# apple/swift-homomorphic-encryption

Measured on NVIDIA H100. Metric: BFV ct*ct mults/sec at N=8192, 4 coefficient moduli, higher is better.
Workload: dtype u64

## Files before the change

### swift-homomorphic-encryption_b200/csrc/ntt_fast.cu

```cuda
#include <cuda.h>

#include <mutex>

#include <algorithm>
#include "kernels.cuh"
#include "ntt_fast.cuh"

namespace hecuda {
using namespace fast;

constexpr int kMaxRowList = 2 * (kMaxL + 1) * kMaxL;
struct RowList {
    int rows_per_poly;
    int count;
    unsigned short row[kMaxRowList];
    unsigned short slot[kMaxRowList];
    unsigned char flags[kMaxRowList];
    unsigned short src_row[kMaxRowList];
    long long src_poly_stride;
};

__device__ __forceinline__ u32 smem_u32(const void *p) { return (u32)__cvta_generic_to_shared(p); }
__device__ __forceinline__ void mbar_init(u64 *bar, int count) {
    asm volatile("mbarrier.init.shared::cta.b64 [%0], %1;" ::"r"(smem_u32(bar)), "r"(count) : "memory");
    asm volatile("fence.mbarrier_init.release.cluster;" ::: "memory");
}
__device__ __forceinline__ void mbar_arrive_expect_tx(u64 *bar, u32 bytes) {
    asm volatile("mbarrier.arrive.expect_tx.shared::cta.b64 _, [%0], %1;" ::"r"(smem_u32(bar)), "r"(bytes) : "memory");
}
__device__ __forceinline__ void mbar_wait(u64 *bar, u32 parity) {
    asm volatile(
        "{\n\t.reg .pred done;\n\t"
        "WAIT_%=:\n\t"
        "mbarrier.try_wait.parity.shared::cta.b64 done, [%0], %1;\n\t"
        "@!done bra WAIT_%=;\n\t}" ::"r"(smem_u32(bar)),
        "r"(parity)
        : "memory");
}
__device__ __forceinline__ void tma_load_1d(void *smem_dst, const void *gmem_src, u32 bytes, u64 *bar) {
    asm volatile("cp.async.bulk.shared::cluster.global.mbarrier::complete_tx::bytes [%0], [%1], %2, [%3];" ::"r"(smem_u32(smem_dst)),
                 "l"(gmem_src), "r"(bytes), "r"(smem_u32(bar))
                 : "memory");
}
__device__ __forceinline__ void tma_load_box(void *smem_dst, const CUtensorMap *map, int line, u64 *bar) {
    asm volatile("cp.async.bulk.tensor.2d.shared::cluster.global.tile.mbarrier::complete_tx::bytes [%0], [%1, {%2, %3}], [%4];" ::"r"(
                     smem_u32(smem_dst)),
                 "l"(map), "r"(0), "r"(line), "r"(smem_u32(bar))
                 : "memory");
}
__device__ __forceinline__ void tma_store_box(const CUtensorMap *map, int line, const void *smem_src) {
    asm volatile("cp.async.bulk.tensor.2d.global.shared::cta.tile.bulk_group [%0, {%1, %2}], [%3];" ::"l"(map), "r"(0), "r"(line),
                 "r"(smem_u32(smem_src))
                 : "memory");
}
__device__ __forceinline__ void tma_prefetch_box(const CUtensorMap *map, int line) {
    asm volatile("cp.async.bulk.prefetch.tensor.2d.L2.global.tile [%0, {%1, %2}];" ::"l"(map), "r"(0), "r"(line) : "memory");
}
__device__ __forceinline__ void tma_commit() { asm volatile("cp.async.bulk.commit_group;" ::: "memory"); }
template <int PENDING>
__device__ __forceinline__ void tma_store_wait_read() { asm volatile("cp.async.bulk.wait_group.read %0;" ::"n"(PENDING) : "memory"); }
__device__ __forceinline__ void tma_store_wait_all() { asm volatile("cp.async.bulk.wait_group 0;" ::: "memory"); }
__device__ __forceinline__ void fence_proxy_async_smem() { asm volatile("fence.proxy.async.shared::cta;" ::: "memory"); }

template <int LOGN, int CLS, int K>
__device__ __forceinline__ void fwd_row_pass(u64 (&x)[16], u64 *sm, int tau, const RowMod &m, bool reduce_in) {
    constexpr int P = plan_passes(LOGN), C = fwd_c(LOGN, K), LB = fwd_lb(LOGN, K);
    load_smem<LOGN, LB, C>(x, sm, tau);
    if (K == 0 && reduce_in) {
#pragma unroll
        for (int r = 0; r < 16; ++r) x[r] = barrett64(x[r], 0 - m.np, m.slot->mu1);
    }
    fwd_pass<LOGN, LB, C, CLS>(x, tau, m);
    if (K == P - 1) fwd_finish<CLS>(x, m);
    store_smem<LOGN, LB, C>(x, sm, tau);
}
template <int LOGN, int CLS>
__device__ __forceinline__ void fwd_row(u64 *sm, int tau, const RowMod &m, bool reduce_in) {
    constexpr int P = plan_passes(LOGN);
    u64 x[16];
    fwd_row_pass<LOGN, CLS, 0>(x, sm, tau, m, reduce_in);
    __syncthreads();
    fwd_row_pass<LOGN, CLS, 1>(x, sm, tau, m, false);
    __syncthreads();
    if (P == 4) {
        fwd_row_pass<LOGN, CLS, (P == 4 ? 2 : 1)>(x, sm, tau, m, false);
        __syncthreads();
    }
    fwd_row_pass<LOGN, CLS, P - 1>(x, sm, tau, m, false);
}

template <int LOGN, int CLS, int K>
__device__ __forceinline__ void inv_row_pass(u64 (&x)[16], u64 *sm, int tau, const RowMod &m) {
    constexpr int C = inv_c(LOGN, K), LB = inv_lb(LOGN, K);
    load_smem<LOGN, LB, C>(x, sm, tau);
    if (narrow_like(CLS) && K > 0 && inv_reduce_at(LOGN, K)) inv_reduce(x, m);
    inv_pass<LOGN, LB, C, CLS, inv_bound_in(LOGN, K)>(x, tau, m);
    if (K == plan_passes(LOGN) - 1 && m.partial) {
        if (CLS == kSmall) {
#pragma unroll
            for (int r = 0; r < 16; ++r) x[r] = csub32((u32)x[r], (u32)(0 - m.np));
        } else {
            reduce_small16(x, m);
        }
    }
    store_smem<LOGN, LB, C>(x, sm, tau);
}
template <int LOGN, int CLS>
__device__ __forceinline__ void inv_row(u64 *sm, int tau, const RowMod &m) {
    constexpr int P = plan_passes(LOGN);
    u64 x[16];
    inv_row_pass<LOGN, CLS, 0>(x, sm, tau, m);
    __syncthreads();
    inv_row_pass<LOGN, CLS, 1>(x, sm, tau, m);
    __syncthreads();
    if (P == 4) {
        inv_row_pass<LOGN, CLS, (P == 4 ? 2 : 1)>(x, sm, tau, m);
        __syncthreads();
    }
    inv_row_pass<LOGN, CLS, P - 1>(x, sm, tau, m);
}

template <int LOGN, unsigned CLASSES>
__device__ __forceinline__ void fwd_row_of(int cls, u64 *sm, int tau, const RowMod &m, bool reduce_in) {
    if (has_class(CLASSES, kNarrowH) && cls == kNarrowH) fwd_row<LOGN, kNarrowH>(sm, tau, m, reduce_in);
    else if (has_class(CLASSES, kNarrow) && narrow_like(cls)) fwd_row<LOGN, kNarrow>(sm, tau, m, reduce_in);
    else if (has_class(CLASSES, kSmall) && cls == kSmall) fwd_row<LOGN, kSmall>(sm, tau, m, reduce_in);
    else if (has_class(CLASSES, kMid) && cls == kMid) fwd_row<LOGN, kMid>(sm, tau, m, reduce_in);
    else if (has_class(CLASSES, kWide)) fwd_row<LOGN, kWide>(sm, tau, m, reduce_in);
}
template <int LOGN, unsigned CLASSES>
__device__ __forceinline__ void inv_row_of(int cls, u64 *sm, int tau, const RowMod &m) {
    if (has_class(CLASSES, kNarrowH) && cls == kNarrowH) inv_row<LOGN, kNarrowH>(sm, tau, m);
    else if (has_class(CLASSES, kNarrow) && narrow_like(cls)) inv_row<LOGN, kNarrow>(sm, tau, m);
    else if (has_class(CLASSES, kSmall) && cls == kSmall) inv_row<LOGN, kSmall>(sm, tau, m);
    else if (has_class(CLASSES, kMid) && cls == kMid) inv_row<LOGN, kMid>(sm, tau, m);
    else if (has_class(CLASSES, kWide)) inv_row<LOGN, kWide>(sm, tau, m);
}

HE_HD constexpr int ntt_row_buffers(int logn) { return logn == 13 ? 2 : 1; }

template <int LOGN>
constexpr size_t ntt_smem_bytes() {
    constexpr int B = ntt_row_buffers(LOGN);
    return sizeof(u64) * B * ((size_t)1 << LOGN) + sizeof(ulonglong2) * ((size_t)1 << (LOGN - 4)) + sizeof(u64) * (B + 1);
}

constexpr int ntt_min_ctas(int logn) { return logn == 13 ? 1 : 1024 / ((1 << logn) / 16); }

template <int LOGN, bool INVERSE, unsigned CLASSES>
__global__ void __launch_bounds__((1 << LOGN) / 16, ntt_min_ctas(LOGN))
    ntt_rows_kernel(const __grid_constant__ CUtensorMap map_in, const __grid_constant__ CUtensorMap map_out,
                    const ModSlot *__restrict__ slots, const __grid_constant__ RowList rl, const int polys,
                    const int scale_mode) {
    extern __shared__ __align__(1024) u64 smem[];
    constexpr int kLines = (1 << LOGN) / kLineWords;
    constexpr int kBoxes = kLines > kBoxLines ? kLines / kBoxLines : 1;
    constexpr int kLinesPerBox = kLines / kBoxes;
    constexpr u32 kRowBytes = (u32)sizeof(u64) << LOGN, kTwBytes = (u32)sizeof(ulonglong2) << (LOGN - 4);
    constexpr int B = ntt_row_buffers(LOGN), AHEAD = B > 1 ? 1 : 0;
    ulonglong2 *tw_cache = reinterpret_cast<ulonglong2 *>(smem + B * (1 << LOGN));
    u64 *bar_row = reinterpret_cast<u64 *>(tw_cache + (1 << (LOGN - 4)));
    u64 *bar_tw = bar_row + B;
    const int tau = threadIdx.x;
    const int tasks = polys * rl.count;
    auto in_line = [&](int t) {
        const int w = t / polys, p = t - w * polys;
        const int64_t word = INVERSE ? ((int64_t)p * rl.rows_per_poly + rl.row[w]) << LOGN
                                     : (int64_t)p * rl.src_poly_stride + ((int64_t)rl.src_row[w] << LOGN);
        return (int)(word >> 4);
    };
    auto load_row = [&](int t, int buf) {
        mbar_arrive_expect_tx(&bar_row[buf], kRowBytes);
        const int line = in_line(t);
        u64 *dst = smem + buf * (1 << LOGN);
#pragma unroll
        for (int b = 0; b < kBoxes; ++b) tma_load_box(dst + b * kLinesPerBox * kLineWords, &map_in, line + b * kLinesPerBox, &bar_row[buf]);
    };
    if (tau == 0) {
        if (smem_u32(smem) & 1023) __trap();
#pragma unroll
        for (int b = 0; b < B; ++b) mbar_init(&bar_row[b], 1);
        mbar_init(bar_tw, 1);
        if (AHEAD && (int)blockIdx.x < tasks) load_row(blockIdx.x, 0);
    }
    __syncthreads();
    u32 phase_row = 0, phase_tw = 0;
    int cached_slot = -1;
    int buf = 0;
    for (int task = blockIdx.x; task < tasks; task += gridDim.x) {
        const int which = task / polys;
        const int poly = task - which * polys;
        const int flags = rl.flags[which];
        const int slot = rl.slot[which];
        const ModSlot &S = slots[slot];
        u64 *sm = smem + buf * (1 << LOGN);
        const int64_t out_word = ((int64_t)poly * rl.rows_per_poly + rl.row[which]) << LOGN;
        const bool new_slot = slot != cached_slot;
        cached_slot = slot;
        if (tau == 0) {
            if (new_slot) {
                mbar_arrive_expect_tx(bar_tw, kTwBytes);
                tma_load_1d(tw_cache, INVERSE ? S.itw : S.tw, kTwBytes, bar_tw);
            }
            const int fill = task + AHEAD * gridDim.x;
            if (fill < tasks) {
                tma_store_wait_read<B - 1 - AHEAD>();
                load_row(fill, (buf + AHEAD) % B);
            }
            const int next = fill + gridDim.x;
            if (next < tasks) {
                const int line = in_line(next);
#pragma unroll
                for (int b = 0; b < kBoxes; ++b) tma_prefetch_box(&map_in, line + b * kLinesPerBox);
            }
        }
        const int cls = flags & 7;
        RowMod m;
        m.np = 0 - S.p;
        m.kp = (cls == kWide || cls == kSmall) ? 2 * S.p : 4 * S.p;
        m.tw = nullptr;
        m.tw_s = smem_u32(tw_cache);
        m.slot = &S;
        m.scale_mode = INVERSE ? scale_mode : -1;
        m.partial = INVERSE && (flags & 16) != 0;
        if (new_slot) {
            mbar_wait(bar_tw, phase_tw);
            phase_tw ^= 1;
        }
        mbar_wait(&bar_row[buf], (phase_row >> buf) & 1);
        phase_row ^= 1u << buf;
        if (INVERSE) inv_row_of<LOGN, CLASSES>(cls, sm, tau, m);
        else fwd_row_of<LOGN, CLASSES>(cls, sm, tau, m, (flags & 8) != 0);
        fence_proxy_async_smem();
        __syncthreads();
        if (tau == 0) {
            const int line = (int)(out_word >> 4);
#pragma unroll
            for (int b = 0; b < kBoxes; ++b) tma_store_box(&map_out, line + b * kLinesPerBox, sm + b * kLinesPerBox * kLineWords);
            tma_commit();
        }
        buf = buf + 1 == B ? 0 : buf + 1;
    }
    if (tau == 0) tma_store_wait_all();
}

__device__ __forceinline__ u32 cluster_ctarank() {
    u32 r;
    asm("mov.u32 %0, %%cluster_ctarank;" : "=r"(r));
    return r;
}
__device__ __forceinline__ int cluster_id_x() {
    u32 r;
    asm("mov.u32 %0, %%clusterid.x;" : "=r"(r));
    return (int)r;
}
__device__ __forceinline__ int cluster_count_x() {
    u32 r;
    asm("mov.u32 %0, %%nclusterid.x;" : "=r"(r));
    return (int)r;
}
__device__ __forceinline__ void cluster_arrive() { asm volatile("barrier.cluster.arrive.release.aligned;" ::: "memory"); }
__device__ __forceinline__ void cluster_wait() { asm volatile("barrier.cluster.wait.acquire.aligned;" ::: "memory"); }
__device__ __forceinline__ void cluster_arrive_relaxed() { asm volatile("barrier.cluster.arrive.relaxed.aligned;" ::: "memory"); }
__device__ __forceinline__ u32 cluster_map(u32 addr, u32 rank) {
    u32 r;
    asm volatile("mapa.shared::cluster.u32 %0, %1, %2;" : "=r"(r) : "r"(addr), "r"(rank));
    return r;
}
__device__ __forceinline__ ulonglong2 ld_cluster_v2(u32 addr) {
    ulonglong2 v;
    asm volatile("ld.shared::cluster.v2.u64 {%0, %1}, [%2];" : "=l"(v.x), "=l"(v.y) : "r"(addr) : "memory");
    return v;
}
template <bool H>
__device__ __forceinline__ u64 mont_product(u64 a, u64 b, u64 p, u64 ninv) { return csub(mont_reduce_c<H>((u128)a * b, p, ninv), p); }

template <int LOGN>
constexpr size_t ntt_tensor_smem_bytes() {
    return sizeof(u64) * 2 * ((size_t)1 << LOGN) + sizeof(ulonglong2) * ((size_t)1 << (LOGN - 4)) + sizeof(u64) * 3;
}

template <int LOGN, bool H>
__device__ __forceinline__ void tensor_step(const u64 *x, const u64 *y, u64 *out, int64_t comp, u32 rank, int tau, u64 p, u64 ninv) {
    constexpr int N = 1 << LOGN, T = N / 16;
    u64 *own = out + (rank ? 2 * comp : 0);
#pragma unroll 4
    for (int w = 2 * tau; w < N; w += 2 * T) {
        const ulonglong2 a = *reinterpret_cast<const ulonglong2 *>(x + w), b = *reinterpret_cast<const ulonglong2 *>(y + w);
        *reinterpret_cast<ulonglong2 *>(own + smem_phys(w)) =
            make_ulonglong2(mont_product<H>(a.x, b.x, p, ninv), mont_product<H>(a.y, b.y, p, ninv));
    }
    cluster_wait();
    const u32 px = cluster_map(smem_u32(x), rank ^ 1), py = cluster_map(smem_u32(y), rank ^ 1);
#pragma unroll 4
    for (int w = (int)rank * (N / 2) + 2 * tau; w < ((int)rank + 1) * (N / 2); w += 2 * T) {
        const ulonglong2 a = *reinterpret_cast<const ulonglong2 *>(x + w), b = *reinterpret_cast<const ulonglong2 *>(y + w);
        const ulonglong2 A = ld_cluster_v2(px + 8u * w), Bv = ld_cluster_v2(py + 8u * w);
        u128 m0 = (u128)a.x * Bv.x, m1 = (u128)a.y * Bv.y;
        mac128(m0, A.x, b.x);
        mac128(m1, A.y, b.y);
        *reinterpret_cast<ulonglong2 *>(out + comp + smem_phys(w)) =
            make_ulonglong2(csub(mont_reduce_c<H>(m0, p, ninv), p), csub(mont_reduce_c<H>(m1, p, ninv), p));
    }
}

template <int LOGN, unsigned CLASSES>
__global__ void __launch_bounds__((1 << LOGN) / 16, 1)
    ntt_forward_tensor_kernel(const __grid_constant__ CUtensorMap map_lhs, const __grid_constant__ CUtensorMap map_rhs,
                              const __grid_constant__ CUtensorMap map_ext, u64 *__restrict__ ten,
                              const ModSlot *__restrict__ slots, const __grid_constant__ RowList rl, const int items,
                              const int L) {
    extern __shared__ __align__(1024) u64 smem[];
    constexpr int N = 1 << LOGN;
    constexpr int kBoxes = N / kLineWords / kBoxLines;
    constexpr u32 kRowBytes = (u32)sizeof(u64) << LOGN, kTwBytes = (u32)sizeof(ulonglong2) << (LOGN - 4);
    static_assert(kBoxes >= 1, "one row is at least one box");
    ulonglong2 *tw_cache = reinterpret_cast<ulonglong2 *>(smem + 2 * N);
    u64 *bar_row = reinterpret_cast<u64 *>(tw_cache + N / 16);
    u64 *bar_tw = bar_row + 2;
    const int tau = threadIdx.x;
    const u32 rank = cluster_ctarank();
    const int first = cluster_id_x(), stride = cluster_count_x();
    const int R = rl.rows_per_poly;
    const int tasks = items * rl.count;
    auto load_row = [&](int t, int j) {
        const int w = t / items, item = t - w * items, r = rl.row[w];
        const CUtensorMap *map;
        int64_t word;
        if (r < L) {
            map = j ? &map_rhs : &map_lhs;
            word = ((int64_t)(2 * item + (int)rank) * L + r) << LOGN;
        } else {
            map = &map_ext;
            word = ((int64_t)(4 * item + 2 * j + (int)rank) * (L + 1) + r - L) << LOGN;
        }
        const int line = (int)(word >> 4);
        mbar_arrive_expect_tx(&bar_row[j], kRowBytes);
#pragma unroll
        for (int b = 0; b < kBoxes; ++b) tma_load_box(smem + j * N + b * kBoxLines * kLineWords, map, line + b * kBoxLines, &bar_row[j]);
    };
    if (tau == 0) {
        if (smem_u32(smem) & 1023) __trap();
        mbar_init(&bar_row[0], 1);
        mbar_init(&bar_row[1], 1);
        mbar_init(bar_tw, 1);
    }
    cluster_arrive();
    cluster_wait();
    u32 phase_row = 0, phase_tw = 0;
    int cached_slot = -1;
    for (int task = first; task < tasks; task += stride) {
        if (task != first) cluster_wait();
        const int which = task / items;
        const int item = task - which * items;
        const int slot = rl.slot[which], r = rl.row[which], cls = rl.flags[which] & 7;
        const ModSlot &S = slots[slot];
        const bool new_slot = slot != cached_slot;
        cached_slot = slot;
        if (tau == 0) {
            if (new_slot) {
                mbar_arrive_expect_tx(bar_tw, kTwBytes);
                tma_load_1d(tw_cache, S.tw, kTwBytes, bar_tw);
            }
            load_row(task, 0);
            load_row(task, 1);
        }
        RowMod m;
        m.np = 0 - S.p;
        m.kp = (cls == kWide || cls == kSmall) ? 2 * S.p : 4 * S.p;
        m.tw = nullptr;
        m.tw_s = smem_u32(tw_cache);
        m.slot = &S;
        m.scale_mode = -1;
        m.partial = false;
        if (new_slot) {
            mbar_wait(bar_tw, phase_tw);
            phase_tw ^= 1;
        }
#pragma unroll
        for (int j = 0; j < 2; ++j) {
            mbar_wait(&bar_row[j], phase_row);
            fwd_row_of<LOGN, CLASSES>(cls, smem + j * N, tau, m, false);
        }
        phase_row ^= 1;
        __syncthreads();
        cluster_arrive();
        const int64_t comp = (int64_t)R * N;
        u64 *out = ten + ((int64_t)3 * item * R + r) * N;
        if (has_class(CLASSES, kNarrowH) && cls == kNarrowH) tensor_step<LOGN, true>(smem, smem + N, out, comp, rank, tau, S.p, S.ninv);
        else tensor_step<LOGN, false>(smem, smem + N, out, comp, rank, tau, S.p, S.ninv);
        fence_proxy_async_smem();
        cluster_arrive_relaxed();
    }
    if (first < tasks) cluster_wait();
}

static void build_row_list(const Context &ctx, const NttRowMap &map, bool inverse, RowList &rl) {
    rl.rows_per_poly = map.rows_per_poly;
    rl.count = 0;
    rl.src_poly_stride = map.src_mod ? map.src_poly_stride : (long long)map.rows_per_poly * ctx.n;
    static const int order[5] = {kWide, kMid, kNarrow, kNarrowH, kSmall};
    for (int oi = 0; oi < 5; ++oi) {
        const int cls = order[oi];
        for (int r = 0; r < map.rows_per_poly; ++r) {
            const int slot = map.slot[r / map.group];
            if (class_of_modulus(ctx.slots[slot].dev.p, ctx.slots[slot].dev.bits) != cls) continue;
            const int i = rl.count++;
            rl.row[i] = (unsigned short)r;
            rl.slot[i] = (unsigned short)slot;
            rl.src_row[i] = (unsigned short)(map.src_mod && !inverse ? r % map.src_mod : r);
            int flags = cls;
            if (map.src_mod && !inverse) {
                const u64 p = ctx.slots[slot].dev.p, src_p = ctx.slots[map.src_slot[r % map.src_mod]].dev.p;
                const u64 room = narrow_like(cls) ? 2u : cls == kMid ? 8u : cls == kSmall ? 1u : 4u;
                if (src_p > p && (src_p - 1) / p >= room) flags |= 8;
            }
            rl.flags[i] = (unsigned char)flags;
        }
    }
}

typedef CUresult (*EncodeTiledFn)(CUtensorMap *, CUtensorMapDataType, cuuint32_t, void *, const cuuint64_t *, const cuuint64_t *,
                                  const cuuint32_t *, const cuuint32_t *, CUtensorMapInterleave, CUtensorMapSwizzle,
                                  CUtensorMapL2promotion, CUtensorMapFloatOOBfill);
static EncodeTiledFn encode_tiled() {
    static EncodeTiledFn fn = [] {
        void *p = nullptr;
        cudaDriverEntryPointQueryResult q;
        if (cudaGetDriverEntryPoint("cuTensorMapEncodeTiled", &p, cudaEnableDefault, &q) != cudaSuccess || q != cudaDriverEntryPointSuccess)
            p = nullptr;
        return (EncodeTiledFn)p;
    }();
    return fn;
}
static bool make_line_map(CUtensorMap *map, const u64 *base, int logn) {
    EncodeTiledFn enc = encode_tiled();
    if (!enc || (reinterpret_cast<uintptr_t>(base) & 15)) return false;
    const int lines = (1 << logn) / kLineWords;
    const cuuint64_t dims[2] = {kLineWords, (cuuint64_t)1 << 31};
    const cuuint64_t strides[1] = {kLineWords * sizeof(u64)};
    const cuuint32_t box[2] = {kLineWords, (cuuint32_t)(lines > kBoxLines ? kBoxLines : lines)};
    const cuuint32_t elem_strides[2] = {1, 1};
    return enc(map, CU_TENSOR_MAP_DATA_TYPE_UINT64, 2, const_cast<u64 *>(base), dims, strides, box, elem_strides,
               CU_TENSOR_MAP_INTERLEAVE_NONE, CU_TENSOR_MAP_SWIZZLE_128B, CU_TENSOR_MAP_L2_PROMOTION_L2_128B,
               CU_TENSOR_MAP_FLOAT_OOB_FILL_NONE) == CUDA_SUCCESS;
}

static bool narrow_h_rows(const RowList &rl) {
    bool any_h = false;
    for (int i = 0; i < rl.count; ++i) {
        const int cls = rl.flags[i] & 7;
        if (!narrow_like(cls)) return false;
        any_h |= cls == kNarrowH;
    }
    return any_h;
}

template <int LOGN, bool INVERSE, unsigned CLASSES>
static cudaError_t launch_rows(const Context &ctx, const RowList &rl, const u64 *in, u64 *out, int polys, int64_t rows,
                               int scale_mode, cudaStream_t stream) {
    CUtensorMap map_in, map_out;
    if (!make_line_map(&map_in, in, LOGN) || !make_line_map(&map_out, out, LOGN)) return cudaErrorInvalidValue;
    constexpr int threads = (1 << LOGN) / 16;
    constexpr size_t smem = ntt_smem_bytes<LOGN>();
    auto k = ntt_rows_kernel<LOGN, INVERSE, CLASSES>;
    static int ctas_per_sm[64] = {0};
    static std::mutex mu;
    int per_sm;
    {
        std::lock_guard<std::mutex> lock(mu);
        int &c = ctas_per_sm[ctx.device & 63];
        if (c == 0) {
            cudaError_t e;
            if ((e = cudaFuncSetAttribute(k, cudaFuncAttributeMaxDynamicSharedMemorySize, (int)smem)) != cudaSuccess) return e;
            int n = 0;
            if ((e = cudaOccupancyMaxActiveBlocksPerMultiprocessor(&n, k, threads, smem)) != cudaSuccess) return e;
            if (n < 1) return cudaErrorInvalidConfiguration;
            c = n;
        }
        per_sm = c;
    }
    const int64_t grid = std::min<int64_t>(rows, (int64_t)ctx.sm_count * per_sm);
    ++g_kernel_launches;
    k<<<(unsigned)grid, threads, smem, stream>>>(map_in, map_out, ctx.d_slots, rl, polys, scale_mode);
    return cudaGetLastError();
}

template <int LOGN, bool INVERSE>
static cudaError_t launch_logn(const Context &ctx, const NttRowMap &map, const u64 *in, u64 *out, int64_t rows,
                               int scale_mode, cudaStream_t stream) {
    if (rows % map.rows_per_poly) return cudaErrorInvalidValue;
    if (rows == 0) return cudaSuccess;
    if (rows > 0x7fffffffLL) return cudaErrorInvalidValue;
    RowList rl;
    build_row_list(ctx, map, INVERSE, rl);
    if (rl.src_poly_stride % kLineWords) return cudaErrorInvalidValue;
    const int polys = (int)(rows / map.rows_per_poly);
    if (LOGN == 13 && narrow_h_rows(rl))
        return launch_rows<LOGN, INVERSE, (LOGN == 13 ? kNarrowClasses : kAllClasses)>(ctx, rl, in, out, polys, rows, scale_mode, stream);
    return launch_rows<LOGN, INVERSE, kAllClasses>(ctx, rl, in, out, polys, rows, scale_mode, stream);
}

struct SplitRows {
    int rows_per_poly, count;
    unsigned short row[kMaxRowList];
    unsigned short src_row[kMaxRowList], slot[kMaxRowList];
    unsigned char reduce_in[kMaxRowList];
    long long src_poly_stride;
};
__global__ void __launch_bounds__(256) ntt_split_forward_kernel(const u64 *__restrict__ in, u64 *__restrict__ out,
                                                               const ModSlot *__restrict__ slots,
                                                               const __grid_constant__ SplitRows sr, int polys, int logn) {
    const int64_t n = (int64_t)1 << logn, half = n >> 1;
    const int which = blockIdx.y;
    const int64_t poly = blockIdx.z;
    const int64_t i = ((int64_t)blockIdx.x * blockDim.x + threadIdx.x) * 2;
    if (i >= half) return;
    const ModSlot &S = slots[sr.slot[which]];
    const u64 p = S.p;
    const ulonglong2 w = S.tw[1];
    const u64 *src = in + poly * sr.src_poly_stride + ((int64_t)sr.src_row[which] << logn) + i;
    u64 *dst = out + (((poly * sr.rows_per_poly) + sr.row[which]) << logn) + i;
    ulonglong2 x = *reinterpret_cast<const ulonglong2 *>(src), y = *reinterpret_cast<const ulonglong2 *>(src + half);
    if (sr.reduce_in[which]) {
        x.x = barrett64(x.x, p, S.mu1), x.y = barrett64(x.y, p, S.mu1);
        y.x = barrett64(y.x, p, S.mu1), y.y = barrett64(y.y, p, S.mu1);
    }
    const u64 v0 = shoup_mul(y.x, w.x, w.y, p), v1 = shoup_mul(y.y, w.x, w.y, p);
    *reinterpret_cast<ulonglong2 *>(dst) = make_ulonglong2(add_mod(x.x, v0, p), add_mod(x.y, v1, p));
    *reinterpret_cast<ulonglong2 *>(dst + half) = make_ulonglong2(sub_mod(x.x, v0, p), sub_mod(x.y, v1, p));
}
__global__ void __launch_bounds__(256) ntt_merge_inverse_kernel(u64 *__restrict__ data, const ModSlot *__restrict__ slots,
                                                               const __grid_constant__ SplitRows sr, int polys, int logn,
                                                               int scale_mode) {
    const int64_t n = (int64_t)1 << logn, half = n >> 1;
    const int which = blockIdx.y;
    const int64_t poly = blockIdx.z;
    const int64_t i = ((int64_t)blockIdx.x * blockDim.x + threadIdx.x) * 2;
// ... 144 lines not shown
```

### swift-homomorphic-encryption_b200/csrc/ntt_fast.cuh

```cuda
#pragma once
#include "context.hpp"
#include "modarith.cuh"

namespace hecuda {
namespace fast {

constexpr int kMinLogN = 10, kMaxLogN = 14;
constexpr int kSplitLogN = 15;
constexpr int kNarrowBits = 55;
constexpr int kMidBits = 61;
constexpr int kSmallBits = 30;
enum { kNarrow = 0, kMid = 1, kWide = 2, kSmall = 3, kNarrowH = 4 };
HE_HD constexpr int class_of_bits(int bits) {
    return bits <= kSmallBits ? kSmall : bits <= kNarrowBits ? kNarrow : bits <= kMidBits ? kMid : kWide;
}
HE_HD constexpr int class_of_modulus(u64 p, int bits) {
    return (class_of_bits(bits) == kNarrow && (u32)p == 1u) ? kNarrowH : class_of_bits(bits);
}
HE_HD constexpr bool narrow_like(int cls) { return cls == kNarrow || cls == kNarrowH; }

HE_HD constexpr unsigned class_bit(int cls) { return 1u << cls; }
constexpr unsigned kAllClasses = (1u << kNarrow) | (1u << kMid) | (1u << kWide) | (1u << kSmall);
constexpr unsigned kNarrowClasses = (1u << kNarrow) | (1u << kNarrowH);
HE_HD constexpr bool has_class(unsigned set, int cls) { return (set & class_bit(cls)) != 0; }

HE_HD constexpr int plan_passes(int logn) { return logn <= 12 ? 3 : 4; }
HE_HD constexpr int plan_c(int logn, int k) {
    return logn == 10   ? (k == 2 ? 4 : 3)
           : logn == 11 ? (k == 1 ? 3 : 4)
           : logn == 12 ? 4
           : logn == 13 ? (k == 3 ? 4 : 3)
                        : (k == 0 || k == 3 ? 4 : 3);
}
HE_HD constexpr int fwd_c(int logn, int k) { return plan_c(logn, k); }
HE_HD constexpr int fwd_lb(int logn, int k) {
    int s0 = 0;
    for (int i = 0; i < k; ++i) s0 += plan_c(logn, i);
    return logn - s0 - plan_c(logn, k);
}
HE_HD constexpr int inv_c(int logn, int k) { return plan_c(logn, plan_passes(logn) - 1 - k); }
HE_HD constexpr int inv_lb(int logn, int k) {
    int u0 = 0;
    for (int i = 0; i < k; ++i) u0 += inv_c(logn, i);
    return u0;
}
HE_HD constexpr int pass_e(int lb, int c) { return lb == 0 ? 0 : 4 - c; }

HE_HD constexpr int inv_stage_bound(int b) { return 2 * b > 4 ? 2 * b : 4; }
HE_HD constexpr int inv_bound_after(int b, int stages) {
    for (int i = 0; i < stages; ++i) b = inv_stage_bound(b);
    return b;
}
HE_HD constexpr bool inv_pass_fits(int b, int stages) {
    for (int i = 0; i < stages; ++i) {
        if (b > 256) return false;
        b = inv_stage_bound(b);
    }
    return true;
}
HE_HD constexpr bool inv_reduce_at(int logn, int k) {
    int b = 1;
    bool red = false;
    for (int i = 0; i <= k; ++i) {
        const int c = inv_c(logn, i);
        red = !inv_pass_fits(b, c);
        if (red) b = 1;
        b = inv_bound_after(b, c);
    }
    return red;
}
HE_HD constexpr int inv_bound_in(int logn, int k) {
    int b = 1;
    for (int i = 0; i <= k; ++i) {
        const int c = inv_c(logn, i);
        if (!inv_pass_fits(b, c)) b = 1;
        if (i < k) b = inv_bound_after(b, c);
    }
    return b;
}

HE_HD constexpr int smem_phys(int e) { return e ^ (((e >> 4) & 7) << 1); }
HE_HD constexpr int smem_words(int logn) { return 1 << logn; }
constexpr int kLineWords = 16;
constexpr int kBoxLines = 256;

HE_HD ulonglong2 ld_tw(const ulonglong2 *p) {
#if defined(__CUDA_ARCH__)
    return __ldg(p);
#else
    return *p;
#endif
}

template <int LOGN, int LB, int C>
HE_HD int elem_index(int tau, int r) {
    constexpr int E = pass_e(LB, C);
    const int lo = tau & ((1 << (LB - E)) - 1), hi = tau >> (LB - E);
    return (hi << (LB + C)) | ((r >> E) << LB) | (lo << E) | (r & ((1 << E) - 1));
}
template <int LB, int C>
HE_HD constexpr int reg_offset(int r) {
    return ((r >> pass_e(LB, C)) << LB) | (r & ((1 << pass_e(LB, C)) - 1));
}
template <int LB, int C>
HE_HD constexpr bool pass_vec() { return pass_e(LB, C) >= 1 || LB == 0; }

template <int LB, int C>
HE_HD int reg_word(int base_phys, int r) {
    constexpr int kSwizzled = 0x7e;
    const int off = reg_offset<LB, C>(r);
    return (off & kSwizzled) ? (base_phys ^ smem_phys(off)) : (base_phys + off);
}

template <int LOGN, int LB, int C>
HE_HD void load_smem(u64 (&x)[16], const u64 *sm, int tau) {
    const int b = smem_phys(elem_index<LOGN, LB, C>(tau, 0));
    if (pass_vec<LB, C>()) {
#pragma unroll
        for (int r = 0; r < 16; r += 2) {
            const ulonglong2 v = *reinterpret_cast<const ulonglong2 *>(sm + reg_word<LB, C>(b, r));
            x[r] = v.x;
            x[r + 1] = v.y;
        }
    } else {
#pragma unroll
        for (int r = 0; r < 16; ++r) x[r] = sm[reg_word<LB, C>(b, r)];
    }
}
template <int LOGN, int LB, int C>
HE_HD void store_smem(const u64 (&x)[16], u64 *sm, int tau) {
    const int b = smem_phys(elem_index<LOGN, LB, C>(tau, 0));
    if (pass_vec<LB, C>()) {
#pragma unroll
        for (int r = 0; r < 16; r += 2)
            *reinterpret_cast<ulonglong2 *>(sm + reg_word<LB, C>(b, r)) = make_ulonglong2(x[r], x[r + 1]);
    } else {
#pragma unroll
        for (int r = 0; r < 16; ++r) sm[reg_word<LB, C>(b, r)] = x[r];
    }
}

struct RowMod {
    u64 np;
    u64 kp;
    const ulonglong2 *tw;
    unsigned tw_s;
    const ModSlot *slot;
    int scale_mode;
    bool partial;
    HE_HD const ulonglong2 *tw_t() const { return scale_mode < 0 ? slot->tw_t : slot->itw_t; }
};
HE_HD ulonglong2 ld_tw_cached(const RowMod &m, int index) {
#if defined(__CUDA_ARCH__)
    ulonglong2 v;
    asm volatile("ld.shared.v2.u64 {%0, %1}, [%2];" : "=l"(v.x), "=l"(v.y) : "r"(m.tw_s + (unsigned)index * 16u));
    return v;
#else
    return m.tw[index];
#endif
}
HE_HD u64 ld_u64(const u64 *p) {
#if defined(__CUDA_ARCH__)
    return __ldg(p);
#else
    return *p;
#endif
}

HE_HD u64 pack64(u32 lo, u32 hi) {
#if defined(__CUDA_ARCH__)
    u64 v;
    asm("mov.b64 %0, {%1, %2};" : "=l"(v) : "r"(lo), "r"(hi));
    return v;
#else
    return ((u64)hi << 32) | lo;
#endif
}
HE_HD void unpack64(u64 v, u32 &lo, u32 &hi) {
#if defined(__CUDA_ARCH__)
    asm("mov.b64 {%0, %1}, %2;" : "=r"(lo), "=r"(hi) : "l"(v));
#else
    lo = (u32)v;
    hi = (u32)(v >> 32);
#endif
}
HE_HD u64 mul_wide_u32(u32 a, u32 b) {
#if defined(__CUDA_ARCH__)
    u64 d;
    asm("mul.wide.u32 %0, %1, %2;" : "=l"(d) : "r"(a), "r"(b));
    return d;
#else
    return (u64)a * b;
#endif
}
HE_HD u64 mad_wide_u32(u32 a, u32 b, u64 c) {
#if defined(__CUDA_ARCH__)
    u64 d;
    asm("mad.wide.u32 %0, %1, %2, %3;" : "=l"(d) : "r"(a), "r"(b), "l"(c));
    return d;
#else
    return (u64)a * b + c;
#endif
}
HE_HD u32 mul_hi_u32(u32 a, u32 b) {
#if defined(__CUDA_ARCH__)
    return __umulhi(a, b);
#else
    return (u32)(((u64)a * b) >> 32);
#endif
}

HE_HD u64 shoup4(u64 y, u64 w, u64 wp, u64 np) {
#if defined(__CUDA_ARCH__)
    u64 v;
    asm volatile("{\n\t"
        ".reg .u32 y0, y1, w0, w1, p0, p1, n0, n1, a1, b1, q0, q1, v0, v1, z;\n\t"
        ".reg .u64 A, B, Q, V;\n\t"
        "mov.b64 {y0, y1}, %1;\n\t"
        "mov.b64 {w0, w1}, %2;\n\t"
        "mov.b64 {p0, p1}, %3;\n\t"
        "mov.b64 {n0, n1}, %4;\n\t"
        "mul.hi.u32 a1, y1, p0;\n\t"
        "mul.hi.u32 b1, y0, p1;\n\t"
        "mov.u32 z, 0;\n\t"
        "mov.b64 A, {a1, z};\n\t"
        "mov.b64 B, {b1, z};\n\t"
        "mad.wide.u32 Q, y1, p1, A;\n\t"
        "add.u64 Q, Q, B;\n\t"
        "mov.b64 {q0, q1}, Q;\n\t"
        "mul.wide.u32 V, y0, w0;\n\t"
        "mad.wide.u32 V, q0, n0, V;\n\t"
        "mov.b64 {v0, v1}, V;\n\t"
        "mad.lo.u32 v1, y1, w0, v1;\n\t"
        "mad.lo.u32 v1, y0, w1, v1;\n\t"
        "mad.lo.u32 v1, q1, n0, v1;\n\t"
        "mad.lo.u32 v1, q0, n1, v1;\n\t"
        "mov.b64 %0, {v0, v1};\n\t}"
        : "=l"(v)
        : "l"(y), "l"(w), "l"(wp), "l"(np));
    return v;
#else
    const u32 y0 = (u32)y, y1 = (u32)(y >> 32), wp0 = (u32)wp, wp1 = (u32)(wp >> 32);
    const u64 q = (u64)y1 * wp1 + (((u64)y1 * wp0) >> 32) + (((u64)y0 * wp1) >> 32);
    return y * w + q * np;
#endif
}
HE_HD u64 shoup4h(u64 y, u64 w, u64 wp, u64 np) {
#if defined(__CUDA_ARCH__)
    u64 v;
    asm volatile("{\n\t"
        ".reg .u32 y0, y1, w0, w1, p0, p1, n0, n1, nh, a1, b1, q0, q1, v0, v1, z;\n\t"
        ".reg .u64 A, B, Q, V;\n\t"
// ... 27 lines not shown
    const u64 h = (0 - np) >> 32;
    return y * w - q - ((u64)((u32)q * (u32)h) << 32);
#endif
}
template <int CLS>
HE_HD u64 shoup4c(u64 y, u64 w, u64 wp, u64 np) { return CLS == kNarrowH ? shoup4h(y, w, wp, np) : shoup4(y, w, wp, np); }
HE_HD u64 shoup2(u64 y, u64 w, u64 wp, u64 np) { return y * w + mulhi64(y, wp) * np; }

HE_HD u64 reduce_small(u64 x, const u64 p, const u64 np, const int red_shift, const u32 red_recip) {
    const u32 xs = (u32)(x >> red_shift);
    const u32 qhat = mul_hi_u32(xs, red_recip);
    u32 np0, np1, rl, rh;
    unpack64(np, np0, np1);
    unpack64(mad_wide_u32(qhat, np0, x), rl, rh);
    rh = qhat * np1 + rh;
    return csub(pack64(rl, rh), p);
}
HE_HD void reduce_small16(u64 (&x)[16], const RowMod &m) {
    const int shift = m.slot->red_shift;
    const u32 recip = m.slot->red_recip;
    const u64 p = 0 - m.np;
#pragma unroll
    for (int r = 0; r < 16; ++r) x[r] = reduce_small(x[r], p, m.np, shift, recip);
}

HE_HD u32 csub32(u32 x, u32 m) {
    const u32 d = x - m;
    return d < x ? d : x;
}
HE_HD u32 shoup32(u32 y, u32 w, u32 wp, u32 p) {
    return y * w - mul_hi_u32(y, wp) * p;
}

template <int CLS>
HE_HD void ct_butterfly(u64 &x, u64 &y, const ulonglong2 w, const RowMod &m) {
    if (CLS == kSmall) {
        const u32 p = (u32)(0 - m.np), p2 = 2 * p;
        const u32 xr = csub32((u32)x, p2);
        const u32 v = shoup32((u32)y, (u32)w.x, (u32)(w.y >> 32), p);
        x = xr + v;
        y = xr - v + p2;
    } else if (narrow_like(CLS)) {
        const u64 v = shoup4c<CLS>(y, w.x, w.y, m.np);
        const u64 xo = x + v;
        y = x - v + m.kp;
        x = xo;
    } else if (CLS == kMid) {
        const u64 xr = csub(x, m.kp);
        const u64 v = shoup4(y, w.x, w.y, m.np);
        x = xr + v;
        y = xr - v + m.kp;
    } else {
        const u64 xr = csub(x, m.kp);
        const u64 v = shoup2(y, w.x, w.y, m.np);
        x = xr + v;
        y = xr - v + m.kp;
    }
}

template <int LOGN, int LB, int C, int CLS, int J>
HE_HD void fwd_stage(u64 (&x)[16], int tau, const RowMod &m) {
    constexpr int E = pass_e(LB, C), F = 1 << E, S0 = LOGN - LB - C, T = (1 << LOGN) / 16;
    constexpr int H = 1 << (C - 1 - J);
    const int hi = tau >> (LB - E);
    const ulonglong2 *tw_t = LB == 0 ? m.tw_t() + tau : nullptr;
#pragma unroll
    for (int grp = 0; grp < (1 << J); ++grp) {
        const ulonglong2 w = LB == 0 ? ld_tw(tw_t + ((1 << J) - 1 + grp) * T)
                                     : ld_tw_cached(m, (1 << (S0 + J)) + (hi << J) + grp);
#pragma unroll
        for (int k = 0; k < H; ++k) {
            const int a = grp * 2 * H + k;
#pragma unroll
            for (int f = 0; f < F; ++f) ct_butterfly<CLS>(x[a * F + f], x[(a + H) * F + f], w, m);
        }
    }
}
template <int LOGN, int LB, int C, int CLS>
HE_HD void fwd_pass(u64 (&x)[16], int tau, const RowMod &m) {
    fwd_stage<LOGN, LB, C, CLS, 0>(x, tau, m);
    if (C > 1) fwd_stage<LOGN, LB, C, CLS, (C > 1 ? 1 : 0)>(x, tau, m);
    if (C > 2) fwd_stage<LOGN, LB, C, CLS, (C > 2 ? 2 : 0)>(x, tau, m);
    if (C > 3) fwd_stage<LOGN, LB, C, CLS, (C > 3 ? 3 : 0)>(x, tau, m);
}

template <int CLS>
HE_HD void fwd_finish(u64 (&x)[16], const RowMod &m) {
    if (CLS == kSmall) {
        const u32 p = (u32)(0 - m.np);
#pragma unroll
        for (int r = 0; r < 16; ++r) x[r] = csub32(csub32((u32)x[r], 2 * p), p);
    } else {
        reduce_small16(x, m);
    }
}

template <int CLS>
HE_HD void gs_butterfly(u64 &x, u64 &y, const ulonglong2 w, const RowMod &m, u64 kp) {
    if (CLS == kSmall) {
        const u32 p = (u32)(0 - m.np), p2 = 2 * p;
        const u32 s = csub32((u32)x + (u32)y, p2);
        y = shoup32((u32)x - (u32)y + p2, (u32)w.x, (u32)(w.y >> 32), p);
        x = s;
    } else if (narrow_like(CLS)) {
        const u64 s = x + y;
        y = shoup4c<CLS>(x - y + kp, w.x, w.y, m.np);
        x = s;
    } else if (CLS == kMid) {
        const u64 s = csub(x + y, kp);
        y = shoup4(x - y + kp, w.x, w.y, m.np);
        x = s;
    } else {
        const u64 s = csub(x + y, kp);
        y = shoup2(x - y + kp, w.x, w.y, m.np);
        x = s;
    }
}

template <int LOGN, int LB, int C, int CLS, int BIN, int J>
HE_HD void inv_stage(u64 (&x)[16], const int tau, const RowMod &m) {
    constexpr int E = pass_e(LB, C), F = 1 << E, T = (1 << LOGN) / 16;
    constexpr int HH = 1 << J;
    constexpr bool kLast = (LB + J == LOGN - 1);
    constexpr int kGroups = 1 << (LOGN - 1 - LB - J);
    const int hi = tau >> (LB - E);
    const u64 kp = narrow_like(CLS) ? (0 - m.np) * (u64)inv_bound_after(BIN, J) : m.kp;
    const ulonglong2 *tw_t = LB == 0 ? m.tw_t() + tau : nullptr;
#pragma unroll
    for (int grp = 0; grp < (1 << (C - 1 - J)); ++grp) {
        if (!kLast || m.partial) {
            const ulonglong2 w = LB == 0 ? ld_tw(tw_t + (16 - (16 >> J) + grp) * T)
                                         : ld_tw_cached(m, kGroups + (hi << (C - 1 - J)) + grp);
#pragma unroll
            for (int k = 0; k < HH; ++k) {
                const int a = grp * 2 * HH + k;
#pragma unroll
                for (int f = 0; f < F; ++f) gs_butterfly<CLS>(x[a * F + f], x[(a + HH) * F + f], w, m, kp);
            }
        } else {
            const u64 *sc = &m.slot->inv_scale[m.scale_mode].c0;
            const u64 c0 = ld_u64(sc), c0p = ld_u64(sc + 1), c1 = ld_u64(sc + 2), c1p = ld_u64(sc + 3);
#pragma unroll
            for (int k = 0; k < HH; ++k) {
                const int a = grp * 2 * HH + k;
#pragma unroll
                for (int f = 0; f < F; ++f) {
                    if (CLS == kSmall) {
                        const u32 p = (u32)(0 - m.np);
                        const u32 xa = (u32)x[a * F + f], ya = (u32)x[(a + HH) * F + f];
                        x[a * F + f] = csub32(shoup32(xa + ya, (u32)c0, (u32)(c0p >> 32), p), p);
                        x[(a + HH) * F + f] = csub32(shoup32(xa - ya + 2 * p, (u32)c1, (u32)(c1p >> 32), p), p);
                        continue;
                    }
                    const u64 xa = x[a * F + f], ya = x[(a + HH) * F + f];
                    const u64 s = xa + ya;
                    const u64 d = xa - ya + kp;
                    x[a * F + f] = csub(shoup2(s, c0, c0p, m.np), 0 - m.np);
                    x[(a + HH) * F + f] = csub(shoup2(d, c1, c1p, m.np), 0 - m.np);
                }
            }
        }
    }
}

template <int LOGN, int LB, int C, int CLS, int BIN>
HE_HD void inv_pass(u64 (&x)[16], int tau, const RowMod &m) {
    inv_stage<LOGN, LB, C, CLS, BIN, 0>(x, tau, m);
    if (C > 1) inv_stage<LOGN, LB, C, CLS, BIN, (C > 1 ? 1 : 0)>(x, tau, m);
    if (C > 2) inv_stage<LOGN, LB, C, CLS, BIN, (C > 2 ? 2 : 0)>(x, tau, m);
    if (C > 3) inv_stage<LOGN, LB, C, CLS, BIN, (C > 3 ? 3 : 0)>(x, tau, m);
}

HE_HD void inv_reduce(u64 (&x)[16], const RowMod &m) { reduce_small16(x, m); }

HE_HD int fwd_last_source(int logn, int k, int tau) {
    int j = 0;
    while ((2 << j) - 1 <= k) ++j;
    const int grp = k - ((1 << j) - 1);
    return (1 << (logn - 4 + j)) + (tau << j) + grp;
}
HE_HD int inv_first_source(int logn, int k, int tau) {
    int J = 0;
    while (16 - (16 >> (J + 1)) <= k) ++J;
    const int grp = k - (16 - (16 >> J));
    return (1 << (logn - 1 - J)) + (tau << (3 - J)) + grp;
}

}
}
```

Measured before the change: 176,600.

## Replace block-wide NTT pass barriers with minimal named-barrier groups

Computes at compile time which thread bits each NTT pass's shared-memory exchange depends on and replaces __syncthreads between passes with __syncwarp or named bar.sync over the smallest thread group covering that dependency. The tensor step is reordered so each warp reads only the lines its own threads produced, which allows dropping a block-wide barrier before the cluster arrive. It also changes the inverse final scaling to use a different Shoup variant with two conditional subtractions. This cuts block-wide stalls but depends on the thread-to-line mapping analysis being exactly right, otherwise races can appear.

Result: faster. 181,800, median of 6 (+2.9%).

```diff
diff --git a/swift-homomorphic-encryption_b200/csrc/ntt_fast.cu b/swift-homomorphic-encryption_b200/csrc/ntt_fast.cu
--- a/swift-homomorphic-encryption_b200/csrc/ntt_fast.cu
+++ b/swift-homomorphic-encryption_b200/csrc/ntt_fast.cu
@@ -62,6 +62,14 @@
 __device__ __forceinline__ void tma_store_wait_all() { asm volatile("cp.async.bulk.wait_group 0;" ::: "memory"); }
 __device__ __forceinline__ void fence_proxy_async_smem() { asm volatile("fence.proxy.async.shared::cta;" ::: "memory"); }
 
+template <int LOGN, int GROUP>
+__device__ __forceinline__ void pass_sync(int tau) {
+    constexpr int T = (1 << LOGN) / 16;
+    if (GROUP <= 32) __syncwarp();
+    else if (GROUP >= T) __syncthreads();
+    else asm volatile("bar.sync %0, %1;" ::"r"(1 + tau / GROUP), "n"(GROUP) : "memory");
+}
+
 template <int LOGN, int CLS, int K>
 __device__ __forceinline__ void fwd_row_pass(u64 (&x)[16], u64 *sm, int tau, const RowMod &m, bool reduce_in) {
     constexpr int P = plan_passes(LOGN), C = fwd_c(LOGN, K), LB = fwd_lb(LOGN, K);
@@ -79,12 +87,12 @@
     constexpr int P = plan_passes(LOGN);
     u64 x[16];
     fwd_row_pass<LOGN, CLS, 0>(x, sm, tau, m, reduce_in);
-    __syncthreads();
+    pass_sync<LOGN, fwd_sync_threads(LOGN, 0)>(tau);
     fwd_row_pass<LOGN, CLS, 1>(x, sm, tau, m, false);
-    __syncthreads();
+    pass_sync<LOGN, fwd_sync_threads(LOGN, 1)>(tau);
     if (P == 4) {
         fwd_row_pass<LOGN, CLS, (P == 4 ? 2 : 1)>(x, sm, tau, m, false);
-        __syncthreads();
+        pass_sync<LOGN, fwd_sync_threads(LOGN, P == 4 ? 2 : 1)>(tau);
     }
     fwd_row_pass<LOGN, CLS, P - 1>(x, sm, tau, m, false);
 }
@@ -110,12 +118,12 @@
     constexpr int P = plan_passes(LOGN);
     u64 x[16];
     inv_row_pass<LOGN, CLS, 0>(x, sm, tau, m);
-    __syncthreads();
+    pass_sync<LOGN, inv_sync_threads(LOGN, 0)>(tau);
     inv_row_pass<LOGN, CLS, 1>(x, sm, tau, m);
-    __syncthreads();
+    pass_sync<LOGN, inv_sync_threads(LOGN, 1)>(tau);
     if (P == 4) {
         inv_row_pass<LOGN, CLS, (P == 4 ? 2 : 1)>(x, sm, tau, m);
-        __syncthreads();
+        pass_sync<LOGN, inv_sync_threads(LOGN, P == 4 ? 2 : 1)>(tau);
     }
     inv_row_pass<LOGN, CLS, P - 1>(x, sm, tau, m);
 }
@@ -282,10 +290,13 @@
 
 template <int LOGN, bool H>
 __device__ __forceinline__ void tensor_step(const u64 *x, const u64 *y, u64 *out, int64_t comp, u32 rank, int tau, u64 p, u64 ninv) {
-    constexpr int N = 1 << LOGN, T = N / 16;
+    constexpr int N = 1 << LOGN, T = N / 16, kWarpWords = 32 * kLineWords;
+    static_assert(fwd_lb(LOGN, plan_passes(LOGN) - 1) == 0, "the last forward pass gives thread tau line tau");
     u64 *own = out + (rank ? 2 * comp : 0);
+    __syncwarp();
+    const int w0 = (tau / 32) * kWarpWords;
 #pragma unroll 4
-    for (int w = 2 * tau; w < N; w += 2 * T) {
+    for (int w = w0 + 2 * (tau % 32); w < w0 + kWarpWords; w += 64) {
         const ulonglong2 a = *reinterpret_cast<const ulonglong2 *>(x + w), b = *reinterpret_cast<const ulonglong2 *>(y + w);
         *reinterpret_cast<ulonglong2 *>(own + smem_phys(w)) =
             make_ulonglong2(mont_product<H>(a.x, b.x, p, ninv), mont_product<H>(a.y, b.y, p, ninv));
@@ -383,7 +394,6 @@
             fwd_row_of<LOGN, CLASSES>(cls, smem + j * N, tau, m, false);
         }
         phase_row ^= 1;
-        __syncthreads();
         cluster_arrive();
         const int64_t comp = (int64_t)R * N;
         u64 *out = ten + ((int64_t)3 * item * R + r) * N;
diff --git a/swift-homomorphic-encryption_b200/csrc/ntt_fast.cuh b/swift-homomorphic-encryption_b200/csrc/ntt_fast.cuh
--- a/swift-homomorphic-encryption_b200/csrc/ntt_fast.cuh
+++ b/swift-homomorphic-encryption_b200/csrc/ntt_fast.cuh
@@ -45,6 +45,33 @@
     return u0;
 }
 HE_HD constexpr int pass_e(int lb, int c) { return lb == 0 ? 0 : 4 - c; }
+
+HE_HD constexpr int pass_tau_bit(int lb, int c, int i) {
+    return i < pass_e(lb, c) ? -1 : i < lb ? i - pass_e(lb, c) : i < lb + c ? -1 : i - c - pass_e(lb, c);
+}
+HE_HD constexpr int sync_span(int logn, int lb0, int c0, int lb1, int c1) {
+    int h = -1;
+    for (int i = 0; i < logn; ++i) {
+        const int a = pass_tau_bit(lb0, c0, i), b = pass_tau_bit(lb1, c1, i);
+        const int m = a > b ? a : b;
+        if (a != b && m > h) h = m;
+    }
+    return 1 << (h + 1);
+}
+constexpr int kNamedBarriers = 15;
+HE_HD constexpr int sync_group(int logn, int span) {
+    const int t = (1 << logn) / 16;
+    if (span <= 32) return 32;
+    int g = span;
+    while (g < t && t / g > kNamedBarriers) g *= 2;
+    return g < t ? g : t;
+}
+HE_HD constexpr int fwd_sync_threads(int logn, int k) {
+    return sync_group(logn, sync_span(logn, fwd_lb(logn, k), fwd_c(logn, k), fwd_lb(logn, k + 1), fwd_c(logn, k + 1)));
+}
+HE_HD constexpr int inv_sync_threads(int logn, int k) {
+    return sync_group(logn, sync_span(logn, inv_lb(logn, k), inv_c(logn, k), inv_lb(logn, k + 1), inv_c(logn, k + 1)));
+}
 
 HE_HD constexpr int inv_stage_bound(int b) { return 2 * b > 4 ? 2 * b : 4; }
 HE_HD constexpr int inv_bound_after(int b, int stages) {
@@ -431,11 +458,11 @@
                         x[(a + HH) * F + f] = csub32(shoup32(xa - ya + 2 * p, (u32)c1, (u32)(c1p >> 32), p), p);
                         continue;
                     }
-                    const u64 xa = x[a * F + f], ya = x[(a + HH) * F + f];
+                    const u64 xa = x[a * F + f], ya = x[(a + HH) * F + f], p = 0 - m.np;
                     const u64 s = xa + ya;
                     const u64 d = xa - ya + kp;
-                    x[a * F + f] = csub(shoup2(s, c0, c0p, m.np), 0 - m.np);
-                    x[(a + HH) * F + f] = csub(shoup2(d, c1, c1p, m.np), 0 - m.np);
+                    x[a * F + f] = csub(csub(shoup4c<CLS>(s, c0, c0p, m.np), 2 * p), p);
+                    x[(a + HH) * F + f] = csub(csub(shoup4c<CLS>(d, c1, c1p, m.np), 2 * p), p);
                 }
             }
         }
```

## Replace CTA-wide barriers in N=8192 row NTT with group-scoped barriers

Applied to the files above, without the earlier changes.

For LOGN=13, the full __syncthreads between NTT passes is replaced by barriers scoped to only the threads whose data actually moves between passes. These are computed at compile time as a warp sync, a named bar.sync per group, or the full CTA barrier. The final store and the input TMA loads are also split per output group, so each group leader loads and stores only its own boxes, with the mbarrier expecting one arrival per group. The aim is to shorten barrier stalls and let groups overlap their work, at the cost of more complex barrier ID bookkeeping and extra syncs when the twiddle slot changes.

Result: no change. 148,800 before, 150,200 after (median of 6 runs) (+0.9%).

```diff
diff --git a/swift-homomorphic-encryption_b200/csrc/ntt_fast.cu b/swift-homomorphic-encryption_b200/csrc/ntt_fast.cu
--- a/swift-homomorphic-encryption_b200/csrc/ntt_fast.cu
+++ b/swift-homomorphic-encryption_b200/csrc/ntt_fast.cu
@@ -62,6 +62,17 @@
 __device__ __forceinline__ void tma_store_wait_all() { asm volatile("cp.async.bulk.wait_group 0;" ::: "memory"); }
 __device__ __forceinline__ void fence_proxy_async_smem() { asm volatile("fence.proxy.async.shared::cta;" ::: "memory"); }
 
+HE_HD constexpr bool group_barriers(int logn) { return logn == 13; }
+template <int LOGN, bool INV, int K>
+__device__ __forceinline__ void row_barrier(int tau) {
+    if constexpr (group_barriers(LOGN)) pass_barrier<LOGN, INV, K>(tau);
+    else __syncthreads();
+}
+template <int LOGN, bool INV>
+HE_HD constexpr int out_mask() {
+    return group_barriers(LOGN) ? barrier_mask(LOGN, INV, plan_passes(LOGN) - 1) : (1 << tau_bits(LOGN)) - 1;
+}
+
 template <int LOGN, int CLS, int K>
 __device__ __forceinline__ void fwd_row_pass(u64 (&x)[16], u64 *sm, int tau, const RowMod &m, bool reduce_in) {
     constexpr int P = plan_passes(LOGN), C = fwd_c(LOGN, K), LB = fwd_lb(LOGN, K);
@@ -79,12 +90,12 @@
     constexpr int P = plan_passes(LOGN);
     u64 x[16];
     fwd_row_pass<LOGN, CLS, 0>(x, sm, tau, m, reduce_in);
-    __syncthreads();
+    row_barrier<LOGN, false, 0>(tau);
     fwd_row_pass<LOGN, CLS, 1>(x, sm, tau, m, false);
-    __syncthreads();
+    row_barrier<LOGN, false, 1>(tau);
     if (P == 4) {
         fwd_row_pass<LOGN, CLS, (P == 4 ? 2 : 1)>(x, sm, tau, m, false);
-        __syncthreads();
+        row_barrier<LOGN, false, (P == 4 ? 2 : 1)>(tau);
     }
     fwd_row_pass<LOGN, CLS, P - 1>(x, sm, tau, m, false);
 }
@@ -110,12 +121,12 @@
     constexpr int P = plan_passes(LOGN);
     u64 x[16];
     inv_row_pass<LOGN, CLS, 0>(x, sm, tau, m);
-    __syncthreads();
+    row_barrier<LOGN, true, 0>(tau);
     inv_row_pass<LOGN, CLS, 1>(x, sm, tau, m);
-    __syncthreads();
+    row_barrier<LOGN, true, 1>(tau);
     if (P == 4) {
         inv_row_pass<LOGN, CLS, (P == 4 ? 2 : 1)>(x, sm, tau, m);
-        __syncthreads();
+        row_barrier<LOGN, true, (P == 4 ? 2 : 1)>(tau);
     }
     inv_row_pass<LOGN, CLS, P - 1>(x, sm, tau, m);
 }
@@ -163,27 +174,34 @@
     u64 *bar_tw = bar_row + B;
     const int tau = threadIdx.x;
     const int tasks = polys * rl.count;
+    constexpr int kOutMask = out_mask<LOGN, INVERSE>(), kOutGroups = (1 << tau_bits(LOGN)) >> popcount_c(kOutMask);
+    static_assert(kOutMask == (1 << tau_bits(LOGN)) - 1 || (kOutMask & 31) == 31, "an out group is made of whole warps");
+    static_assert(kBoxes % kOutGroups == 0, "every out group writes whole boxes");
+    const bool out_leader = kOutGroups == 1 ? tau == 0 : (tau & kOutMask) == 0;
+    const int out_group = group_of(kOutMask, tau_bits(LOGN), tau);
+    auto my_box = [&](int b) { return kOutGroups == 1 || box_group(LOGN, INVERSE, b) == out_group; };
     auto in_line = [&](int t) {
         const int w = t / polys, p = t - w * polys;
         const int64_t word = INVERSE ? ((int64_t)p * rl.rows_per_poly + rl.row[w]) << LOGN
                                      : (int64_t)p * rl.src_poly_stride + ((int64_t)rl.src_row[w] << LOGN);
         return (int)(word >> 4);
     };
-    auto load_row = [&](int t, int buf) {
-        mbar_arrive_expect_tx(&bar_row[buf], kRowBytes);
+    auto load_boxes = [&](int t, int buf) {
+        mbar_arrive_expect_tx(&bar_row[buf], kRowBytes / kOutGroups);
         const int line = in_line(t);
         u64 *dst = smem + buf * (1 << LOGN);
 #pragma unroll
-        for (int b = 0; b < kBoxes; ++b) tma_load_box(dst + b * kLinesPerBox * kLineWords, &map_in, line + b * kLinesPerBox, &bar_row[buf]);
+        for (int b = 0; b < kBoxes; ++b)
+            if (my_box(b)) tma_load_box(dst + b * kLinesPerBox * kLineWords, &map_in, line + b * kLinesPerBox, &bar_row[buf]);
     };
     if (tau == 0) {
         if (smem_u32(smem) & 1023) __trap();
 #pragma unroll
-        for (int b = 0; b < B; ++b) mbar_init(&bar_row[b], 1);
+        for (int b = 0; b < B; ++b) mbar_init(&bar_row[b], kOutGroups);
         mbar_init(bar_tw, 1);
-        if (AHEAD && (int)blockIdx.x < tasks) load_row(blockIdx.x, 0);
     }
     __syncthreads();
+    if (AHEAD && out_leader && (int)blockIdx.x < tasks) load_boxes(blockIdx.x, 0);
     u32 phase_row = 0, phase_tw = 0;
     int cached_slot = -1;
     int buf = 0;
@@ -197,18 +215,20 @@
         const int64_t out_word = ((int64_t)poly * rl.rows_per_poly + rl.row[which]) << LOGN;
         const bool new_slot = slot != cached_slot;
         cached_slot = slot;
-        if (tau == 0) {
-            if (new_slot) {
+        if (kOutGroups > 1 && new_slot) __syncthreads();
+        if (out_leader) {
+            const bool first = kOutGroups == 1 || tau == 0;
+            if (first && new_slot) {
                 mbar_arrive_expect_tx(bar_tw, kTwBytes);
                 tma_load_1d(tw_cache, INVERSE ? S.itw : S.tw, kTwBytes, bar_tw);
             }
             const int fill = task + AHEAD * gridDim.x;
             if (fill < tasks) {
                 tma_store_wait_read<B - 1 - AHEAD>();
-                load_row(fill, (buf + AHEAD) % B);
+                load_boxes(fill, (buf + AHEAD) % B);
             }
             const int next = fill + gridDim.x;
-            if (next < tasks) {
+            if (first && next < tasks) {
                 const int line = in_line(next);
 #pragma unroll
                 for (int b = 0; b < kBoxes; ++b) tma_prefetch_box(&map_in, line + b * kLinesPerBox);
@@ -232,16 +252,17 @@
         if (INVERSE) inv_row_of<LOGN, CLASSES>(cls, sm, tau, m);
         else fwd_row_of<LOGN, CLASSES>(cls, sm, tau, m, (flags & 8) != 0);
         fence_proxy_async_smem();
-        __syncthreads();
-        if (tau == 0) {
+        row_barrier<LOGN, INVERSE, plan_passes(LOGN) - 1>(tau);
+        if (out_leader) {
             const int line = (int)(out_word >> 4);
 #pragma unroll
-            for (int b = 0; b < kBoxes; ++b) tma_store_box(&map_out, line + b * kLinesPerBox, sm + b * kLinesPerBox * kLineWords);
+            for (int b = 0; b < kBoxes; ++b)
+                if (my_box(b)) tma_store_box(&map_out, line + b * kLinesPerBox, sm + b * kLinesPerBox * kLineWords);
             tma_commit();
         }
         buf = buf + 1 == B ? 0 : buf + 1;
     }
-    if (tau == 0) tma_store_wait_all();
+    if (out_leader) tma_store_wait_all();
 }
 
 __device__ __forceinline__ u32 cluster_ctarank() {
diff --git a/swift-homomorphic-encryption_b200/csrc/ntt_fast.cuh b/swift-homomorphic-encryption_b200/csrc/ntt_fast.cuh
--- a/swift-homomorphic-encryption_b200/csrc/ntt_fast.cuh
+++ b/swift-homomorphic-encryption_b200/csrc/ntt_fast.cuh
@@ -92,12 +92,89 @@
 #endif
 }
 
+HE_HD constexpr int pass_elem(int lb, int c, int tau, int r) {
+    const int e = pass_e(lb, c);
+    const int lo = tau & ((1 << (lb - e)) - 1), hi = tau >> (lb - e);
+    return (hi << (lb + c)) | ((r >> e) << lb) | (lo << e) | (r & ((1 << e) - 1));
+}
 template <int LOGN, int LB, int C>
-HE_HD int elem_index(int tau, int r) {
-    constexpr int E = pass_e(LB, C);
-    const int lo = tau & ((1 << (LB - E)) - 1), hi = tau >> (LB - E);
-    return (hi << (LB + C)) | ((r >> E) << LB) | (lo << E) | (r & ((1 << E) - 1));
-}
+HE_HD constexpr int elem_index(int tau, int r) { return pass_elem(LB, C, tau, r); }
+
+constexpr int kBoxBits = 12;
+HE_HD constexpr int pass_lb(int logn, bool inv, int k) { return inv ? inv_lb(logn, k) : fwd_lb(logn, k); }
+HE_HD constexpr int pass_c(int logn, bool inv, int k) { return inv ? inv_c(logn, k) : fwd_c(logn, k); }
+HE_HD constexpr int tau_bits(int logn) { return logn - 4; }
+HE_HD constexpr int tau_bit_elem(int logn, bool inv, int k, int i) {
+    const int e = pass_elem(pass_lb(logn, inv, k), pass_c(logn, inv, k), 1 << i, 0);
+    int b = 0;
+    while ((e >> b) > 1) ++b;
+    return b;
+}
+HE_HD constexpr int pass_owner(int logn, bool inv, int k, int e) {
+    int tau = 0;
+    for (int i = 0; i < tau_bits(logn); ++i) tau |= ((e >> tau_bit_elem(logn, inv, k, i)) & 1) << i;
+    return tau;
+}
+HE_HD constexpr int barrier_moving_bits(int logn, bool inv, int k) {
+    int m = 0;
+    for (int i = 0; i < tau_bits(logn); ++i) {
+        const int b = tau_bit_elem(logn, inv, k, i);
+        if (k + 1 < plan_passes(logn) ? b != tau_bit_elem(logn, inv, k + 1, i) : b < kBoxBits) m |= 1 << i;
+    }
+    return m;
+}
+HE_HD constexpr int barrier_mask(int logn, bool inv, int k) {
+    const int m = barrier_moving_bits(logn, inv, k);
+    return (m >> 5) ? (m | 31) : m;
+}
+enum { kBarWarp = 0, kBarNamed = 1, kBarCta = 2 };
+HE_HD constexpr int barrier_kind(int logn, bool inv, int k) {
+    return barrier_mask(logn, inv, k) == (1 << tau_bits(logn)) - 1 ? kBarCta : barrier_mask(logn, inv, k) < 32 ? kBarWarp : kBarNamed;
+}
+HE_HD constexpr int popcount_c(int m) {
+    int n = 0;
+    for (; m; m >>= 1) n += m & 1;
+    return n;
+}
+HE_HD constexpr int barrier_threads(int logn, bool inv, int k) { return 1 << popcount_c(barrier_mask(logn, inv, k)); }
+HE_HD constexpr int barrier_groups(int logn, bool inv, int k) { return (1 << tau_bits(logn)) / barrier_threads(logn, inv, k); }
+HE_HD constexpr int group_of(int mask, int nbits, int tau) {
+    int g = 0, j = 0;
+    for (int i = 0; i < nbits; ++i)
+        if (!((mask >> i) & 1)) g |= ((tau >> i) & 1) << j++;
+    return g;
+}
+HE_HD constexpr int barrier_group(int logn, bool inv, int k, int tau) {
+    return group_of(barrier_mask(logn, inv, k), tau_bits(logn), tau);
+}
+HE_HD constexpr int barrier_first_id(int logn, bool inv, int k) {
+    int id = 1;
+    for (int j = 0; j < k; ++j)
+        if (barrier_kind(logn, inv, j) == kBarNamed) id += barrier_groups(logn, inv, j);
+    return id;
+}
+HE_HD constexpr int box_group(int logn, bool inv, int b) {
+    const int k = plan_passes(logn) - 1;
+    return barrier_group(logn, inv, k, pass_owner(logn, inv, k, b << kBoxBits));
+}
+
+#if defined(__CUDACC__)
+template <int LOGN, bool INV, int K>
+__device__ __forceinline__ void pass_barrier(int tau) {
+    constexpr int kKind = barrier_kind(LOGN, INV, K), kMask = barrier_mask(LOGN, INV, K);
+    static_assert(kKind != kBarNamed || (kMask & 31) == 31, "a named barrier joins whole warps");
+    static_assert(kKind != kBarWarp || kMask < 32, "a warp barrier stays inside one warp");
+    static_assert(barrier_first_id(LOGN, INV, plan_passes(LOGN)) <= 16, "named barrier ids are 1..15");
+    if (kKind == kBarCta) {
+        __syncthreads();
+    } else if (kKind == kBarWarp) {
+        __syncwarp();
+    } else {
+        constexpr int kFirst = barrier_first_id(LOGN, INV, K), kThreads = barrier_threads(LOGN, INV, K);
+        asm volatile("bar.sync %0, %1;" ::"r"(kFirst + group_of(kMask, tau_bits(LOGN), tau)), "n"(kThreads) : "memory");
+    }
+}
+#endif
 template <int LB, int C>
 HE_HD constexpr int reg_offset(int r) {
     return ((r >> pass_e(LB, C)) << LB) | (r & ((1 << pass_e(LB, C)) - 1));
```
